# lucanest/Phyloformer

Measured on AMD Instinct MI355X. Metric: alignments/sec, 60-leaf/500-site LG+GC-like MSAs, Phyloformer forward (pf.ckpt), higher is better.
Workload: dtype f16x3-split MFMA (two fp16 limbs per operand, 3 passes), fp32 accumulate/residual

## Files before the change

### include/phyloformer_amd.h

```cpp
#ifndef PHYLOFORMER_AMD_H
#define PHYLOFORMER_AMD_H

#include <stddef.h>
#include <stdint.h>

#ifdef __cplusplus
extern "C" {
#endif

#define PF_ABI_VERSION 5

typedef enum pf_status {
    PF_OK = 0,
    PF_EINVAL = -1,
    PF_EHIP = -2,
    PF_ERCCL = -3,
    PF_ENOMEM = -4,
    PF_ESTATE = -5,
    PF_EIO = -6
} pf_status;

typedef struct pf_weights_t {
    int32_t n_blocks;
    int32_t n_heads;
// ... 73 lines not shown
int pf_bme_spr_host(const float* preds, const int32_t* start_slots, int32_t B, int32_t N, int32_t* slots, double* lengths, int32_t* steps,
                    double* tree_length, uint8_t* status);

int pf_forward_weighted(pf_handle_t* h, const uint8_t* idx, int32_t B, int32_t N, int32_t L, const float* w, float* out);
int pf_forward_weighted_device(pf_handle_t* h, const uint8_t* d_idx, int32_t B, int32_t N, int32_t L, const float* d_w,
                               float* d_out);
int pf_forward_sites_weighted(pf_handle_t* h, const uint8_t* idx, int32_t B, int32_t N, int32_t L, const int32_t* sites,
                              const float* w, int32_t S, int32_t K, float* out);
int pf_bootstrap_weighted(pf_handle_t* h, const uint8_t* idx, int32_t B, int32_t N, int32_t L, int32_t R, uint64_t seed,
                          float* out);
int pf_padded_sites(int32_t K, int32_t L);
int pf_boot_counts(int32_t L, int32_t R, uint64_t seed, int32_t r, int32_t* sites, int32_t* counts);
int pf_compress_sites(const uint8_t* idx, int32_t N, int32_t L, int32_t* first, int32_t* count);

int pf_forward_site_map(pf_handle_t* h, const uint8_t* idx, int32_t B, int32_t N, int32_t L, float* out, float* map);
int pf_forward_site_map_device(pf_handle_t* h, const uint8_t* d_idx, int32_t B, int32_t N, int32_t L, float* d_out,
                               float* d_map);
int pf_forward_site_profile(pf_handle_t* h, const uint8_t* idx, int32_t B, int32_t N, int32_t L, float* out, float* se,
                            float* profile);
int pf_site_moments_device(pf_handle_t* h, const float* d_map, int32_t B, int32_t P, int32_t L, float* d_se,
                           float* d_profile);

int pf_forward_sharded(pf_handle_t* h, const uint8_t* idx, int32_t B, int32_t N,
                       int32_t l_begin, int32_t l_end, int32_t L_total, float* out);
int pf_forward_sharded_device(pf_handle_t* h, const uint8_t* d_idx, int32_t B, int32_t N,
                              int32_t l_begin, int32_t l_end, int32_t L_total, float* d_out);

#define PF_UNIQUE_ID_BYTES 256
int pf_comm_unique_id(void* id_out);
int pf_comm_init(pf_handle_t* h, const void* unique_id, int32_t rank, int32_t world_size);
int pf_comm_destroy(pf_handle_t* h);
int pf_comm_info(char* path_out, size_t path_cap, int32_t* version);

int pf_synchronize(pf_handle_t* h);
int pf_get_stream(pf_handle_t* h, void** hip_stream_out);
int pf_device_malloc(pf_handle_t* h, size_t bytes, void** out);
int pf_device_free(pf_handle_t* h, void* p);
int pf_memcpy_h2d(pf_handle_t* h, void* dst, const void* src, size_t bytes);
int pf_memcpy_d2h(pf_handle_t* h, void* dst, const void* src, size_t bytes);

int pf_profile_reset(pf_handle_t* h);
int pf_profile_get(pf_handle_t* h, const char* kernel, int64_t* launches, double* total_ms);

int64_t pf_debug_read(pf_handle_t* h, const char* name, float* dst, int64_t cap);

int pf_device_info(pf_handle_t* h, char* name_out, size_t name_cap, int32_t* cu_count,
                   uint64_t* hbm_bytes);
int pf_device_pci(pf_handle_t* h, int32_t* domain, int32_t* bus, int32_t* device);

int pf_forward_shards_emulated(pf_handle_t* h, const uint8_t* idx, int32_t B, int32_t N, int32_t L,
                               int32_t nshards, float* out);

int pf_selftest(pf_handle_t* h, float* out);

typedef struct pf_mha_weights_t {
    int32_t n_heads;
    int32_t embed_dim;
    const float *wq, *bq, *wk, *bk, *wv, *bv, *wo, *bo;
} pf_mha_weights_t;
typedef struct pf_mha pf_mha_t;
int pf_create_bare(int device, pf_handle_t** out);
int pf_mha_create(pf_handle_t* h, const pf_mha_weights_t* w, pf_mha_t** out);
int pf_mha_destroy(pf_mha_t* m);
int pf_mha_forward(pf_mha_t* m, const float* x, int32_t B, int32_t R, int32_t C, float* y);
int pf_mha_forward_device(pf_mha_t* m, const float* d_x, int32_t B, int32_t R, int32_t C, float* d_y);

#define PF_FASTA_EBYTE (-16)
#define PF_FASTA_ERAGGED (-17)
#define PF_FASTA_ENOHEADER (-18)
#define PF_FASTA_EEMPTY (-19)
#define PF_FASTA_ECAP (-20)
#define PF_FASTA_EUTF8 (-21)
int pf_parse_fasta(const char* data, int64_t len, uint8_t* idx, int64_t idx_cap, int64_t* id_spans,
                   int32_t max_seqs, int32_t* n_out, int32_t* l_out, int64_t* detail);

int64_t pf_format_phylip(const float* preds, int32_t n, const char* const* ids, char* out, int64_t cap);
int64_t pf_format_phylip_n(const float* preds, int32_t n, const char* const* ids, const int64_t* id_lens, char* out,
                           int64_t cap);

int64_t pf_nj_newick_n(const float* preds, int32_t n, const char* const* ids, const int64_t* id_lens, int32_t clamp_negative,
                       char* out, int64_t cap);

int64_t pf_nj_format_joins_n(const int32_t* slots, const double* lengths, int32_t n, const char* const* ids, const int64_t* id_lens,
                             int32_t clamp_negative, char* out, int64_t cap);

int64_t pf_bme_newick_n(const float* preds, int32_t n, const char* const* ids, const int64_t* id_lens, int32_t clamp_negative,
                        char* out, int64_t cap);

int64_t pf_bme_spr_newick_n(const float* preds, int32_t n, const char* const* ids, const int64_t* id_lens, int32_t clamp_negative,
                            char* out, int64_t cap);

typedef struct pf_fasta_batch pf_fasta_batch_t;
int pf_fasta_batch_load(const char* const* paths, int32_t count, int32_t threads, pf_fasta_batch_t** out);
void pf_fasta_batch_free(pf_fasta_batch_t* b);
int32_t pf_fasta_batch_count(const pf_fasta_batch_t* b);
int pf_fasta_batch_infos(const pf_fasta_batch_t* b, int32_t* status, int32_t* n, int32_t* l, int64_t* detail);
int pf_fasta_batch_id(const pf_fasta_batch_t* b, int32_t file, int32_t seq, const char** id, int64_t* len);
int pf_fasta_batch_gather(const pf_fasta_batch_t* const* batches, const int32_t* file_idx, int32_t count, int32_t n,
                          int32_t l, uint8_t* dst);
int pf_phylip_write_batch(const pf_fasta_batch_t* const* batches, const int32_t* file_idx, int32_t count, int32_t n,
                          const float* preds, const char* const* out_paths, const char* const* tree_paths, int32_t threads,
                          int32_t* status);

#ifdef __cplusplus
}
#endif
// ... 2 lines not shown
```

### phyloformer_amd/csrc/pf_device.hip.h

```cpp
#pragma once
#include <hip/hip_runtime.h>
#include <stdint.h>

#include "pf_layout.h"

namespace pfk {

typedef float f32x4 __attribute__((ext_vector_type(4)));
typedef float f32x16 __attribute__((ext_vector_type(16)));
#if PF_F16
typedef _Float16 h16_t;
#define PF_MFMA(a, b, c) __builtin_amdgcn_mfma_f32_32x32x16_f16((a), (b), (c), 0, 0, 0)
#define PF_DOT2C "v_dot2c_f32_f16"
#define PF_CVT_PK "v_cvt_pk_f16_f32"
#define PF_NEG1_LO 0x0000bc00u
#define PF_NEG1_HI 0xbc000000u
#else
typedef __bf16 h16_t;
#define PF_MFMA(a, b, c) __builtin_amdgcn_mfma_f32_32x32x16_bf16((a), (b), (c), 0, 0, 0)
#define PF_DOT2C "v_dot2c_f32_bf16"
#define PF_CVT_PK "v_cvt_pk_bf16_f32"
#define PF_NEG1_LO 0x0000bf80u
#define PF_NEG1_HI 0xbf800000u
#endif
// ... 342 lines not shown
    const int k0 = (int)(((long)p * L) >> 5), k1 = (int)((((long)p + 1) * L - 1) >> 5);
    *first = (long)b * slots_aln + k0 + p;
    *count = k1 - k0 + 1;
}

template <int LO, int HI>
__device__ __forceinline__ void image_to_lds(const frag_t* src, unsigned char* smem) {
    static_assert(LO % 64 == 0 && HI % 64 == 0, "the image is copied in whole waves");
    const int wv = threadIdx.x >> 6, ln = threadIdx.x & 63;
#pragma unroll
    for (int k = 0; k < (HI - LO + MAIN_THREADS - 1) / MAIN_THREADS; ++k) {
        const int f0 = LO + k * MAIN_THREADS + wv * 64;
        if (f0 < HI) __builtin_amdgcn_global_load_lds(src + f0 + ln, smem + (size_t)f0 * 16, 16, 0, 0);
    }
}

template <int MODE, bool FLAT, bool SITEMAP = false, bool WEIGHTED = false>
__global__ void __launch_bounds__(MAIN_THREADS, MAIN_WAVES / 4) k_main(MainArgs a) {
    constexpr bool LAST = MODE == MODE_LAST || MODE == MODE_LAST_FOLD;
    constexpr bool FOLD = MODE == MODE_LAST_FOLD;
    static_assert(!SITEMAP || LAST, "the site map is the head's: last block only");
    static_assert(!WEIGHTED || (!SITEMAP && MODE != MODE_FIRST), "weighted launches: blocks' own modes, no site map");
    extern __shared__ __attribute__((aligned(16))) unsigned char smem[];
    lds_frag_t lw = (lds_frag_t)smem;
    lds_f32_t lc = (lds_f32_t)(smem + FRAG_END * 16);

    {
        const float cv = a.consts[min((int)threadIdx.x, CONST_LEN - 1)];
        if (FOLD) {
            image_to_lds<FRAG_W1, FRAG_W2>(a.wimg, smem);
            image_to_lds<FRAG_WO, FRAG_U + U_FRAGS>(a.wimg, smem);
        } else {
            image_to_lds<(MODE == MODE_FIRST) ? FRAG_WV : 0, LAST ? FRAG_WV : FRAG_END>(a.wimg, smem);
        }
        static_assert(CONST_LEN <= MAIN_THREADS, "one constant per thread");
        if (threadIdx.x < CONST_LEN) reinterpret_cast<float*>(smem + FRAG_END * 16)[threadIdx.x] = cv;
        asm volatile("s_waitcnt vmcnt(0)" ::: "memory");
    }
    __syncthreads();

    const int lane = threadIdx.x & 63;
    const int wave = __builtin_amdgcn_readfirstlane(threadIdx.x >> 6);
    const int t = lane & 31;
    const int h = lane >> 5;
    const int ntiles = (a.Lloc + 31) >> 5;
    const int ntasks = a.B * a.nt_aln;
    if (wave >= MAIN_WAVES / 2) __builtin_amdgcn_s_setprio(1);
    unsigned long long tacc[6] = {0, 0, 0, 0, 0, 0}, tprev = 0;
#define PF_TICK(k) do { if (a.prof) { const unsigned long long tn_ = __builtin_amdgcn_s_memtime(); tacc[k] += tn_ - tprev; tprev = tn_; } } while (0)
    if (a.prof) tprev = __builtin_amdgcn_s_memtime();
    lds_frag_t w1p = lw + FRAG_W1 + lane;
    lds_frag_t w2p = lw + FRAG_W2 + lane;
    lds_frag_t wop = lw + FRAG_WO + lane;
    lds_frag_t qkp = lw + FRAG_QK + h * 8 + (t & 7);
    lds_f32_t lch = lc + 4 * h;
    PF_OPAQUE(wop); PF_OPAQUE(qkp); PF_OPAQUE(lch);
    lds_frag_t wvp = wop + (FRAG_WV - FRAG_WO);
    lds_f32_t luh = (lds_f32_t)(smem + FRAG_U * 16) + 16 * h;

    {
        const int nwaves = gridDim.x * MAIN_WAVES;
#ifndef PF_RUN_MAX
#define PF_RUN_MAX 8
#endif
        const int run = max(1, min(PF_RUN_MAX, ntasks / (nwaves * 8)));
        int run0 = (blockIdx.x * MAIN_WAVES + wave) * run;
        const int task0 = run0, task1 = ntasks;
        TilePos cur = tile_pos<FLAT>(a, min(task0, ntasks - 1), ntiles);
        int frag_row = -1;
        frag_t mfr[4];
        f32x4 rqv = {0.f, 0.f, 0.f, 0.f};
        f32x4 px[8], pctx[8], pqr, pqc;
        int pri = 0, prj = 0;
        auto prefetch = [&](const TilePos& np) {
            const LanePos nl = lane_pos<FLAT>(a, np, t);
            const int ll = nl.l, pb = np.b;
            const size_t tk = nl.tok0 + nl.toff;
            if (MODE == MODE_MID0) {
                const uint8_t* ib = a.idx + (size_t)pb * a.N * a.Lloc + ll;
                const int pp = np.r0 + (nl.in_r1 ? 1 : 0);
                pri = residue(ib[(size_t)a.pair_i[pp] * a.Lloc]);
                prj = residue(ib[(size_t)a.pair_j[pp] * a.Lloc]);
            } else {
                const f32x4* xp = reinterpret_cast<const f32x4*>(a.x + tk * 64 + 4 * h);
#pragma unroll
                for (int g = 0; g < 8; ++g) px[g] = xp[2 * g];
            }
            pqr = *reinterpret_cast<const f32x4*>(a.qrow + tk * 4);
            pqc = *reinterpret_cast<const f32x4*>(a.qcol + tk * 4);
            if (MODE != MODE_FIRST) {
                int hq = h;
                asm volatile("" : "+v"(hq));
                const f32x4* cp = reinterpret_cast<const f32x4*>(a.ctx + ((size_t)pb * a.Lloc + ll) * 64 + 4 * hq);
#pragma unroll
                for (int g = 0; g < 8; ++g) pctx[g] = cp[2 * g];
            }
        };
        if (MODE != MODE_FIRST && task0 < task1) prefetch(cur);

        for (int task = task0; task < task1;) {
            const int b = cur.b;
            const int row = b * a.P + cur.r0;
            int ntask = task + 1;
            TilePos nxt = tile_next<FLAT>(a, cur);
            if (ntask == run0 + run) {
                run0 += nwaves * run;
                ntask = run0;
                if (ntask < task1) nxt = tile_pos<FLAT>(a, ntask, ntiles);
            }
            const LanePos lp = lane_pos<FLAT>(a, cur, t);
            const bool straddle = lp.wrap < 32;
            int ai = 0, aj = 0;
            if (MODE == MODE_FIRST) { const int pp = cur.r0 + (lp.in_r1 ? 1 : 0); ai = a.pair_i[pp]; aj = a.pair_j[pp]; }
            auto load_mfr = [&](int r) {
                const frag_t* mf = a.mfrag + (size_t)r * 128 + t;
#pragma unroll
                for (int q = 0; q < 4; ++q) mfr[q] = mf[q * 32];
                typedef const f32x4 __attribute__((address_space(4)))* const_f32x4_t;
                rqv = *(const_f32x4_t)(unsigned long long)(a.rq + (size_t)__builtin_amdgcn_readfirstlane(r) * 4);
                frag_row = r;
            };
            if (MODE != MODE_FIRST && row != frag_row) load_mfr(row);
            const bool valid = lp.valid;
            const int lc_ = lp.l;
            const size_t tok = lp.tok0 + lp.toff;
            float x[32];
            float zh[4] = {0.f, 0.f, 0.f, 0.f};
            float wt = 1.f;
            if (WEIGHTED && LAST) wt = a.w[(size_t)b * a.Lloc + lc_];

            if (MODE == MODE_FIRST) {
                const int ri = residue(a.idx[((size_t)b * a.N + ai) * a.Lloc + lc_]);
                const int rj = residue(a.idx[((size_t)b * a.N + aj) * a.Lloc + lc_]);
                const f32x4* ti = reinterpret_cast<const f32x4*>(a.table + ri * 64 + 4 * h);
                const f32x4* tj = reinterpret_cast<const f32x4*>(a.table + rj * 64 + 4 * h);
#pragma unroll
                for (int g = 0; g < 8; ++g) {
                    f32x4 u = ti[2 * g], w = tj[2 * g];
#pragma unroll
                    for (int i = 0; i < 4; ++i) x[4 * g + i] = u[i] + w[i];
                }
            } else {
                if (MODE == MODE_MID0) {
                    const f32x4* ti = reinterpret_cast<const f32x4*>(a.table + pri * 64 + 4 * h);
                    const f32x4* tj = reinterpret_cast<const f32x4*>(a.table + prj * 64 + 4 * h);
#pragma unroll
                    for (int g = 0; g < 8; ++g) {
                        const f32x4 u = ti[2 * g], w = tj[2 * g];
#pragma unroll
                        for (int i = 0; i < 4; ++i) x[4 * g + i] = u[i] + w[i];
                    }
                } else {
#pragma unroll
                    for (int g = 0; g < 8; ++g)
#pragma unroll
                        for (int i = 0; i < 4; ++i) x[4 * g + i] = px[g][i];
                }
                PF_TICK(0);
                if (!(a.ablate & 8)) {
                    f32x16 ya[2];
#pragma unroll
                    for (int j = 0; j < 32; ++j) ya[j >> 4][j & 15] = x[j];
                    {
                        const f32x4 qr = pqr;
                        auto mix = [&](const bool mine) {
                            float v[8];
#pragma unroll
                            for (int i = 0; i < 4; ++i) v[i] = mine ? qr[i] * rqv[i] : 0.f;
                            v[4] = v[5] = mine ? 1.f : 0.f;
                            v[6] = v[7] = 0.f;
                            frag_t qb_hi, qb_lo;
                            split8(v, qb_hi, qb_lo);
#pragma unroll
                            for (int To = 0; To < 2; ++To) mfma3(ya[To], mfr[To * 2], mfr[To * 2 + 1], qb_hi, qb_lo, To == 1);
                        };
                        mix(h == 0 && !lp.in_r1);
                        if (straddle) {
                            load_mfr(row + 1);
                            mix(h == 0 && lp.in_r1);
                        }
                    }
                    {
                        const f32x4 qc = pqc * COLAPPLY_B_SCALE;
                        float o[32];
#pragma unroll
                        for (int g = 0; g < 8; ++g) {
                            const f32x4 u = pctx[g];
#pragma unroll
                            for (int i = 0; i < 4; ++i) o[4 * g + i] = u[i] * qc[g >> 1];
                        }
#pragma unroll
                        for (int s = 0; s < 4; ++s) {
                            frag_t ob_hi, ob_lo;
                            split8(&o[8 * s], ob_hi, ob_lo);
#pragma unroll
                            for (int To = 0; To < 2; ++To) {
                                lds_frag_t f = wop + ((To * 4 + s) * 2) * 64;
                                const frag_t a_hi = f[0], a_lo = f[64];
                                mfma3(ya[To], a_hi, a_lo, ob_hi, ob_lo, To == 1);
                            }
                        }
                    }
#pragma unroll
                    for (int j = 0; j < 32; ++j) x[j] = ya[j >> 4][j & 15];
                }

                PF_TICK(1);
                if (FOLD) {
#pragma unroll
                    for (int g = 0; g < 8; ++g) {
                        const f32x4 w4 = *(lds_f32x4_t)(lch + CONST_HW + 8 * g);
#pragma unroll
                        for (int i = 0; i < 4; ++i) zh[i] = fmaf(w4[i], x[4 * g + i], zh[i]);
                    }
                }
                if (FOLD && !(a.ablate & 16)) {
                    frag_t xb_hi[4], xb_lo[4];
                    {
                        float xn[32];
                        ln_pair(x, xn);
#pragma unroll
                        for (int s = 0; s < 4; ++s) split8(&xn[8 * s], xb_hi[s], xb_lo[s]);
                    }
                    if (ntask < task1) prefetch(nxt);
                    PF_TICK(2);
#pragma unroll 1
                    for (int T = 0; T < 8; ++T) {
                        f32x16 ha;
                        lds_frag_t f1 = w1p + T * 512;
                        lds_f32_t bp = lch + CONST_B1 + 32 * T;
                        lds_f32_t up = luh + 32 * T;
                        PF_OPAQUE(f1); PF_OPAQUE(bp); PF_OPAQUE(up);
// ... 43 lines not shown
                            frag_t nh, nl;
                            if (s < 3) { nh = f1[(s + 1) * 128]; nl = f1[(s + 1) * 128 + 64]; }
                            else { nh = f2[0]; nl = f2[64]; }
                            mfma3(ha, fh, fl, xb_hi[s], xb_lo[s]);
                            fh = nh; fl = nl;
                        }
                        frag_t g_hi[2], g_lo[2];
                        gelu_split8(ha, 0, g_hi[0], g_lo[0]);
                        gelu_split8(ha, 8, g_hi[1], g_lo[1]);
#pragma unroll
                        for (int st = 0; st < 4; ++st) {
                            const int u = st >> 1, To = st & 1;
                            frag_t nh = fh, nl = fl;
                            if (st < 3) {
                                const int nu = (st + 1) >> 1, nTo = (st + 1) & 1;
                                nh = f2[(nTo * 32 + nu * 2) * 64];
                                nl = f2[(nTo * 32 + nu * 2) * 64 + 64];
                            }
                            mfma3(oa[To], fh, fl, g_hi[u], g_lo[u], To == 1);
                            fh = nh; fl = nl;
                        }
                    }
                    PF_TICK(3);
#pragma unroll
                    for (int j = 0; j < 32; ++j) x[j] = oa[j >> 4][j & 15];
                }
            }

            if (!LAST && !(a.ablate & 4)) {
                frag_t wl[8];
#pragma unroll
                for (int i = WVLO_LDS; i < 8; ++i) wl[i] = a.wv_lo[i * 64 + lane];
                if (WEIGHTED) wt = a.w[(size_t)b * a.Lloc + lc_];
                __builtin_amdgcn_sched_barrier(0);
                {
                    const size_t stok = valid ? tok : a.trash_tok + t;
                    f32x4* xo = reinterpret_cast<f32x4*>(a.x + stok * 64 + 4 * h);
#pragma unroll
                    for (int g = 0; g < 8; ++g) {
                        f32x4 u = {x[4 * g], x[4 * g + 1], x[4 * g + 2], x[4 * g + 3]};
                        xo[2 * g] = u;
                    }
                }
                if (a.ablate & 32) { cur = nxt; task = ntask; continue; }
                f32x16 va[3];
                {
                    float xn[32];
                    ln_pair(x, xn);
                    frag_t xb_hi[4], xb_lo[4];
#pragma unroll
                    for (int s = 0; s < 4; ++s) split8(&xn[8 * s], xb_hi[s], xb_lo[s]);
#pragma unroll
                    for (int s = 0; s < 4; ++s) {
                        const frag_t q_hi = qkp[(s * 2) * 16], q_lo = qkp[(s * 2 + 1) * 16];
                        if (s == 0) mfma3_zero(va[2], q_hi, q_lo, xb_hi[s], xb_lo[s]);
                        else mfma3(va[2], q_hi, q_lo, xb_hi[s], xb_lo[s]);
                    }
#pragma unroll
                    for (int s = 0; s < 4; ++s)
#pragma unroll
                        for (int T = 0; T < 2; ++T) {
                            const frag_t f_hi = wvp[(T * 4 + s) * 64];
                            const frag_t f_lo = T * 4 + s < WVLO_LDS ? wvp[(FRAG_WVLO - FRAG_WV) + (T * 4 + s) * 64] : wl[T * 4 + s];
                            if (s == 0) mfma3_zero(va[T], f_hi, f_lo, xb_hi[s], xb_lo[s], T == 1);
                            else mfma3(va[T], f_hi, f_lo, xb_hi[s], xb_lo[s], T == 1);
                        }
                }
#pragma unroll
                for (int r = 0; r < 4; ++r) va[2][r] += lc[CONST_BQK + 4 * h + r];
                float qk[4], ot[4];
#pragma unroll
                for (int i = 0; i < 4; ++i) qk[i] = elu1_fast(va[2][i]);
#pragma unroll
                for (int i = 0; i < 4; ++i) ot[i] = pair_other(qk[i], h);
                float qn[4], kn[4];
#pragma unroll
                for (int i = 0; i < 4; ++i) {
                    qn[i] = h ? ot[i] : qk[i];
                    kn[i] = h ? qk[i] : ot[i];
                }
                {
                    const size_t stok = valid ? tok : a.trash_tok + t;
                    f32x4 qs = {qn[0], qn[1], qn[2], qn[3]};
                    *reinterpret_cast<f32x4*>(a.qrow + stok * 4) = qs;
                }
                const long slot0 = (long)b * a.slots_aln + cur.kt + (FLAT ? cur.r0 : 0);
                for (int part = 0; part < (straddle ? 2 : 1); ++part) {
                    float* sp = a.spart + (size_t)(slot0 + part) * SROW;
                    const float vm = (valid && lp.in_r1 == (part == 1)) ? (WEIGHTED ? wt : 1.f) : 0.f;
                    float km[4];
#pragma unroll
                    for (int i = 0; i < 4; ++i) km[i] = kn[i] * vm;
                    {
                        float qk8[8];
#pragma unroll
                        for (int i = 0; i < 4; ++i) { qk8[i] = vm * qn[i]; qk8[4 + i] = km[i]; }
                        const float sqk = treduce8(qk8, t);
                        if (lane < 8) sp[64 + lane] = sqk;
                    }
                    {
                        float kv[32];
#pragma unroll
                        for (int j = 0; j < 32; ++j) kv[j] = km[j >> 3] * va[j >> 4][j & 15];
                        sp[kmap(t, h)] = treduce32(kv, t);
                    }
                }
            } else if (LAST) {
                float z = 0.f;
                if (FOLD) {
                    z = pair_sum((zh[0] + zh[1]) + (zh[2] + zh[3])) + lc[CONST_C0];
                } else {
#pragma unroll
                    for (int g = 0; g < 8; ++g) {
                        const f32x4 w4 = *(lds_f32x4_t)(lch + CONST_HW + 8 * g);
#pragma unroll
                        for (int i = 0; i < 4; ++i) z = fmaf(w4[i], x[4 * g + i], z);
                    }
                    z = pair_sum(z) + lc[CONST_HB];
                }
                const float spz = softplus20(z);
                const long slot0 = (long)b * a.slots_aln + cur.kt + (FLAT ? cur.r0 : 0);
                for (int part = 0; part < (straddle ? 2 : 1); ++part) {
// ... 178 lines not shown
        const float* sp = a.srow + (size_t)first * SROW;
        const int c2 = 64 + (c & 7);
        float acc = 0.f, acc2 = 0.f;
        for (int i = 0; i < nparts; i += 8) {
            const float* q0 = sp + i * SROW;
            float v[8], w8[8];
#pragma unroll
            for (int q = 0; q < 8; ++q) {
                const bool on = i + q < nparts;
                v[q] = on ? q0[q * SROW + c] : 0.f;
                w8[q] = on ? q0[q * SROW + c2] : 0.f;
            }
#pragma unroll
            for (int q = 0; q < 8; ++q) { acc += v[q]; acc2 += w8[q]; }
        }
        st[sub][c] = acc;
        if (c < 8) st[sub][64 + c] = acc2;
    }
    __syncthreads();
    if (ok) {
        const float* s = st[sub];
        const int hh = c >> 4;
        const float sk = s[68 + hh];
        ctx[sub][c] = (s[c] + bvc * sk) / sk;
        if (c < 4) {
            const float* ws = a.wst ? a.wst + (size_t)(pr / a.P) * 4 : nullptr;
            const float r = (ws ? ws[0] : a.L_total) / s[64 + c];
            rqs[sub][c] = r;
            a.rq[(size_t)pr * 4 + c] = r * (ws ? ws[2] : a.b_scale);
        }
    }
    __syncthreads();
    if (ok) {
        float* m = a.mrow ? a.mrow + (size_t)pr * MROW : nullptr;
#pragma unroll
        for (int hh = 0; hh < 4; ++hh) {
            float acc = 0.f;
#pragma unroll
            for (int d = 0; d < 16; ++d) acc = fmaf(wo[hh][d], ctx[sub][16 * hh + d], acc);
            if (m) m[hh * 64 + c] = acc * rqs[sub][hh];
            mm[sub][hh][c] = acc * (a.wst ? a.wst[(size_t)(pr / a.P) * 4 + 3] : a.a_scale);
        }
        mm[sub][4][c] = biasc;
        mm[sub][5][c] = biascol;
    }
    __syncthreads();
    if (ok) {
        const int To = c >> 5, t = c & 31;
        float v[8];
#pragma unroll
        for (int i = 0; i < 8; ++i) v[i] = (i < 6) ? mm[sub][i][32 * To + t] : 0.f;
        frag_t hi, lo;
        split8(v, hi, lo);
        frag_t* mf = a.mfrag + (size_t)pr * MFRAG_PER_PAIR + To * 64 + t;
        mf[0] = hi;
        mf[32] = lo;
    }
    }
}

__global__ void k_rowsum(const float* spart, float* srow, int npairs, int nparts_, int flat, int P, int Lloc, int slots_aln) {
    const int i = blockIdx.x * blockDim.x + threadIdx.x;
    if (i >= npairs * SROW) return;
    const int pr = i / SROW, c = i - pr * SROW;
    long first;
    int nparts;
    part_range(flat, pr, nparts_, P, Lloc, slots_aln, &first, &nparts);
    const float* sp = spart + (size_t)first * SROW + c;
    float acc = 0.f;
    for (int k = 0; k < nparts; k += 8) {
        float v[8];
#pragma unroll
        for (int q = 0; q < 8; ++q) v[q] = k + q < nparts ? sp[(size_t)(k + q) * SROW] : 0.f;
#pragma unroll
        for (int q = 0; q < 8; ++q) acc += v[q];
    }
    srow[i] = acc;
}

__global__ void k_outsum(const float* outpart, float* out, int npairs, int nparts_, float inv_L_total, int flat, int P,
                         int Lloc, int slots_aln, const float* wst) {
    const int pr = blockIdx.x * blockDim.x + threadIdx.x;
    if (pr >= npairs) return;
    long first;
    int nparts;
    part_range(flat, pr, nparts_, P, Lloc, slots_aln, &first, &nparts);
    const float* sp = outpart + first;
    float acc = 0.f;
    for (int k = 0; k < nparts; k += 8) {
        float v[8];
#pragma unroll
        for (int q = 0; q < 8; ++q) v[q] = k + q < nparts ? sp[k + q] : 0.f;
#pragma unroll
        for (int q = 0; q < 8; ++q) acc += v[q];
    }
    out[pr] = acc * (wst ? wst[(size_t)(pr / P) * 4 + 1] : inv_L_total);
}

struct ColStatsArgs {
    const float* x;
    const float* qrow;
    const float* mrow;
    float* qcol;
    float* part;
    const float* wqk;
    const float* bqk;
    const float* brow;
    int B, P, Lloc, G, nchunks;
    int sub, S, fine;
// ... 333 lines not shown
                    float v[GU][4];
#pragma unroll
                    for (int u = 0; u < GU; ++u)
#pragma unroll
                        for (int q = 0; q < 4; ++q)
                            v[u][q] = s + q < n[u] ? pg[u][(size_t)(s + q) * gs] : 0.f;
#pragma unroll
                    for (int u = 0; u < GU; ++u) t[u] = (((t[u] + v[u][0]) + v[u][1]) + v[u][2]) + v[u][3];
                }
#pragma unroll
                for (int u = 0; u < GU; ++u)
                    if (g + u < a.G) acc += t[u];
            }
        } else {
            const float* pp = a.part + ((size_t)b * a.G * a.Lloc + l) * CPART + i;
            int g = 0;
            for (; g + 4 <= a.G; g += 4) {
                const float v0 = pp[(size_t)g * gs], v1 = pp[(size_t)(g + 1) * gs], v2 = pp[(size_t)(g + 2) * gs],
                            v3 = pp[(size_t)(g + 3) * gs];
                acc = (((acc + v0) + v1) + v2) + v3;
            }
            for (; g < a.G; ++g) acc += pp[(size_t)g * gs];
        }
        zs[i] = acc;
    }
    __syncthreads();
    if (i < 256) {
        const float* z = zs + (hd >> 4) * 64 + 16 * quarter;
        float acc = 0.f;
#pragma unroll
        for (int k = 0; k < 16; ++k) acc = fmaf(w[k], z[k], acc);
        dp[quarter][hd] = acc;
    }
    __syncthreads();
    if (i < 64) {
        const int hh = hd >> 4;
        const float acc = ((dp[0][hd] + dp[1][hd]) + dp[2][hd]) + dp[3][hd];
        const float sq = zs[256 + hh], sk = zs[260 + hh];
        a.ctx[(size_t)site * 64 + hd] = (acc + a.bv[hd] * sk) / sk * (a.P / sq);
    }
}

__global__ void k_accumulate(float* dst, const float* src, size_t n) {
    const size_t i = (size_t)blockIdx.x * blockDim.x + threadIdx.x;
    if (i < n) dst[i] += src[i];
}

__global__ void k_selftest(float* out) {
    const int lane = threadIdx.x;
    out[lane] = pair_sum((float)lane);
    out[64 + lane] = pair_other((float)lane, lane >> 5);
    out[128 + lane] = row16_sum((float)lane);
    out[192 + lane] = half32_sum((float)lane);
    frag_t A1, A2, Bf;
    const int m = lane & 31, kg = lane >> 5;
#pragma unroll
    for (int i = 0; i < 8; ++i) {
        const int k = 8 * kg + i;
        A1[i] = (h16_t)(float)(m + 32 * (k % 8));
        A2[i] = (h16_t)(float)k;
        Bf[i] = (h16_t)((k == (m & 15)) ? 1.f : 0.f);
    }
    f32x16 acc1, acc2;
#pragma unroll
    for (int r = 0; r < 16; ++r) { acc1[r] = 0.f; acc2[r] = 0.f; }
    acc1 = PF_MFMA(A1, Bf, acc1);
    acc2 = PF_MFMA(A2, Bf, acc2);
#pragma unroll
    for (int r = 0; r < 16; ++r) {
        out[256 + lane * 16 + r] = acc1[r];
        out[1280 + lane * 16 + r] = acc2[r];
    }
}

#endif

}
```

### phyloformer_amd/csrc/pf_layout.h

```cpp
#pragma once

#ifndef PF_F16
#define PF_F16 1
#endif

namespace pfk {

constexpr int E = 64;
constexpr int NH = 4;
constexpr int HD = 16;
constexpr int FF = 256;
constexpr int NA = 22;
constexpr int SROW = 72;
constexpr int MROW = 4 * 64;
constexpr float LN_EPS = 1e-5f;

constexpr int FRAG_W1 = 0;
constexpr int FRAG_W2 = FRAG_W1 + 8 * 4 * 2 * 64;
constexpr int FRAG_WO = FRAG_W2 + 2 * 16 * 2 * 64;
constexpr int FRAG_WV = FRAG_WO + 2 * 4 * 2 * 64;
constexpr int FRAG_QK = FRAG_WV + 2 * 4 * 64;
#ifndef PF_WVLO_LDS
#define PF_WVLO_LDS 4
#endif
constexpr int WVLO_LDS = PF_WVLO_LDS;
constexpr int FRAG_WVLO = FRAG_QK + 4 * 2 * 16;
constexpr int FRAG_END = FRAG_WVLO + WVLO_LDS * 64;
constexpr int FRAG_U = FRAG_WV;
constexpr int U_FRAGS = FF * 4 / 16;
static_assert(FRAG_U + U_FRAGS <= FRAG_END, "the folded head fits the last block's tail");
constexpr int WVLO_FRAGS = 2 * 4 * 64;
constexpr int CONST_B1 = 0, CONST_B2 = 256, CONST_BQK = 320, CONST_HW = 328, CONST_HB = 392,
              CONST_C0 = 393, CONST_BOC = 400;
constexpr int CONST_LEN = 464;
constexpr int MAIN_LDS_BYTES = FRAG_END * 16 + CONST_LEN * 4;
constexpr int MFRAG_PER_PAIR = 2 * 2 * 32;

constexpr int MAIN_THREADS = 512;
constexpr int MAIN_WAVES = MAIN_THREADS / 64;

constexpr int PAIRTAB_ROWS = 22 * 22, PAIRTAB_W = 72;

}
```

### phyloformer_amd/csrc/pf_lib.hip

```cpp
#include <hip/hip_runtime.h>
#include <dlfcn.h>

#include <algorithm>
#include <cmath>
#include <cstdarg>
#include <cstdio>
#include <cstdlib>
#include <cstring>
#include <functional>
#include <map>
#include <mutex>
#include <string>
#include <type_traits>
#include <vector>

#include "../../include/phyloformer_amd.h"
#include "pf_device.hip.h"
#include "pf_mha.hip.h"
#include "pf_precise.hip.h"
#include "pf_generic.hip.h"
#include "pf_boot.hip.h"
#include "pf_sites.hip.h"
#include "pf_sitemap.hip.h"
#include "pf_sites_host.h"
// ... 2558 lines not shown
}

int pf_device_pci(pf_handle_t* h, int32_t* domain, int32_t* bus, int32_t* device) {
    if (!h) return PF_EINVAL;
    if (domain) *domain = h->prop.pciDomainID;
    if (bus) *bus = h->prop.pciBusID;
    if (device) *device = h->prop.pciDeviceID;
    return PF_OK;
}

int pf_forward_shards_emulated(pf_handle_t* h, const uint8_t* idx, int32_t B, int32_t N, int32_t L,
                               int32_t nshards, float* out) {
    if (!h) return PF_EINVAL;
    int rc = check_dims(h, B, N, L, L);
    if (rc) return rc;
    if (nshards < 1 || nshards > 64 || !idx || !out) return fail(h, PF_EINVAL, "bad shard count or null buffer");
    HIPCHK(h, hipSetDevice(h->device));
    if (const F64Path* f = f64_path_of(h, N, L)) return forward_shards_emulated_f64(h, *f, idx, B, N, L, nshards, out);
    if ((rc = ensure_pairs(h, N))) return rc;
    const int P = N * (N - 1) / 2;
    ShardStage stage(h);
    if ((rc = stage.upload(idx, B, N, L, nshards))) return rc;
    std::vector<ShardRun> runs;
    for (const ShardStage::Shard& s : stage.shards) {
        ShardRun r{{}, s.d_idx, nullptr, B, N, P, s.Lloc, L, tile_plan(h, P, s.Lloc), h->stream, {}};
        size_t off[WS_BUFS];
        char* ws = (char*)stage.alloc(workspace_bytes(h, B, P, r.Lloc, &r.w, off));
        r.d_out = (float*)stage.alloc((size_t)B * P * sizeof(float));
        if (!ws || !r.d_out) return fail(h, PF_ENOMEM, "shard workspace allocation failed");
        carve_workspace(ws, off, &r.w);
        runs.push_back(r);
    }
    float* total = (float*)stage.alloc((size_t)B * P * SROW * sizeof(float));
    if (!total) return fail(h, PF_ENOMEM, "shard sum buffer");
    auto reduce = [&](bool site_sums) -> int {
        const size_t count = (size_t)B * P * (site_sums ? 1 : SROW);
        for (ShardRun& r : runs)
            if (!site_sums && (rc = launch_rowsum(h, r, &r.rs))) return rc;
        hipMemsetAsync(total, 0, count * sizeof(float), h->stream);
        for (ShardRun& r : runs) {
            hipLaunchKernelGGL(k_accumulate, dim3((unsigned)((count + 255) / 256)), dim3(256), 0, h->stream,
                               total, site_sums ? r.d_out : r.w.srow, count);
            r.rs = RowStats{total, 1, 0};
        }
        return PF_OK;
    };
    rc = schedule(h, runs.data(), runs.size(), reduce);
    if (!rc && (hipMemcpyAsync(out, total, (size_t)B * P * sizeof(float), hipMemcpyDeviceToHost, h->stream) != hipSuccess ||
                hipStreamSynchronize(h->stream) != hipSuccess))
        rc = fail(h, PF_EHIP, "result copy failed");
    return rc;
}

int pf_selftest(pf_handle_t* h, float* out) {
    if (!h || !out) return PF_EINVAL;
    float* d = nullptr;
    HIPCHK(h, hipMalloc((void**)&d, 2304 * sizeof(float)));
    hipLaunchKernelGGL(k_selftest, dim3(1), dim3(64), 0, h->stream, d);
    HIPCHK(h, hipGetLastError());
    HIPCHK(h, hipMemcpyAsync(out, d, 2304 * sizeof(float), hipMemcpyDeviceToHost, h->stream));
    HIPCHK(h, hipStreamSynchronize(h->stream));
    hipFree(d);
    return PF_OK;
}

struct pf_mha {
    pf_handle* h = nullptr;
    float* wfrag = nullptr;
    float* bias = nullptr;
    char* ws = nullptr;
    size_t ws_bytes = 0;
    float* d_x = nullptr;
    float* d_y = nullptr;
    size_t d_xy_bytes = 0;
};

int pf_mha_create(pf_handle_t* h, const pf_mha_weights_t* w, pf_mha_t** out) {
    if (!h || !w || !out) return PF_EINVAL;
    if (w->n_heads != MHA_H || w->embed_dim != E)
        return fail(h, PF_EINVAL, "softmax attention kernels are specialised for embed_dim 64 / 4 heads, got %d / %d",
                    w->embed_dim, w->n_heads);
    const float* ws[4] = {w->wq, w->wk, w->wv, w->wo};
    const float* bs[4] = {w->bq, w->bk, w->bv, w->bo};
    std::vector<uint16_t> img((size_t)MHA_WTOTAL * 8);
    std::vector<float> bias(4 * E);
    for (int i = 0; i < 4; ++i) {
        if (!ws[i] || !bs[i]) return fail(h, PF_EINVAL, "pf_mha_create: NULL weight pointer");
        std::copy(bs[i], bs[i] + E, bias.begin() + i * E);
    }
    pack_frags(w->wq, E, E, E, img.data());
    pack_frags(w->wk, E, E, E, img.data() + (size_t)MHA_OFF_WK * 8);
    pack_frags(w->wv, E, E, E, img.data() + (size_t)MHA_OFF_WV * 8);
    pack_frags(w->wo, E, E, E, img.data() + (size_t)MHA_OFF_WO * 8);
    HIPCHK(h, hipSetDevice(h->device));
    pf_mha* m = new pf_mha();
    m->h = h;
    void* p = nullptr;
    if (hipMalloc(&p, img.size() * 2) != hipSuccess) { delete m; return fail(h, PF_ENOMEM, "pf_mha_create: hipMalloc failed"); }
    m->wfrag = (float*)p;
    if (hipMalloc(&p, bias.size() * 4) != hipSuccess) { hipFree(m->wfrag); delete m; return fail(h, PF_ENOMEM, "pf_mha_create: hipMalloc failed"); }
    m->bias = (float*)p;
    if (hipMemcpy(m->wfrag, img.data(), img.size() * 2, hipMemcpyHostToDevice) != hipSuccess ||
        hipMemcpy(m->bias, bias.data(), bias.size() * 4, hipMemcpyHostToDevice) != hipSuccess) {
        hipFree(m->wfrag); hipFree(m->bias); delete m;
        return fail(h, PF_EHIP, "pf_mha_create: weight upload failed");
    }
    *out = m;
    return PF_OK;
}

int pf_mha_destroy(pf_mha_t* m) {
    if (!m) return PF_OK;
    hipSetDevice(m->h->device);
    hipStreamSynchronize(m->h->stream);
    hipFree(m->wfrag); hipFree(m->bias);
    if (m->ws) hipFree(m->ws);
    if (m->d_x) hipFree(m->d_x);
// ... 82 lines not shown
```

### phyloformer_amd/engine.py

```python
from __future__ import annotations

import ctypes as C
import os
from typing import Dict, Optional, Tuple

import numpy as np

from .weights import ModelWeights

HERE = os.path.dirname(os.path.abspath(__file__))
LIB_PATH = os.path.join(HERE, "libphyloformer_amd.so")
ABI_VERSION = 5
UNIQUE_ID_BYTES = 256

PF_OK, PF_EINVAL, PF_EHIP, PF_ERCCL, PF_ENOMEM, PF_ESTATE = 0, -1, -2, -3, -4, -5


def _refuse_single_sequence(B: int, N: int):
    if N == 1 and B >= 1:
        raise RuntimeError(f"cannot reshape tensor of 0 elements into shape [{B}, -1, 0, 64] because the unspecified "
                           "dimension size -1 can be any value and is ambiguous")


class EngineError(RuntimeError):
# ... 1 lines not shown
    def __init__(self, code: int, msg: str):
        super().__init__(f"[pf status {code}] {msg}")
        self.code = code


class pf_weights_t(C.Structure):
    _fields_ = [("n_blocks", C.c_int32), ("n_heads", C.c_int32), ("embed_dim", C.c_int32),
                ("n_alphabet", C.c_int32), ("blob", C.POINTER(C.c_float)), ("blob_len", C.c_uint64)]


_H = C.c_void_p
SIGNATURES = {
    "pf_abi_version": (C.c_int, []),
    "pf_build_info": (C.c_char_p, []),
    "pf_blob_len": (C.c_uint64, [C.c_int32, C.c_int32, C.c_int32]),
    "pf_create": (C.c_int, [C.POINTER(pf_weights_t), C.c_int, C.POINTER(_H)]),
    "pf_destroy": (C.c_int, [_H]),
    "pf_last_error": (C.c_char_p, [_H]),
    "pf_set_option": (C.c_int, [_H, C.c_char_p, C.c_int64]),
    "pf_forward": (C.c_int, [_H, C.c_void_p, C.c_int32, C.c_int32, C.c_int32, C.c_void_p]),
    "pf_forward_device": (C.c_int, [_H, C.c_void_p, C.c_int32, C.c_int32, C.c_int32, C.c_void_p]),
    "pf_resample_sites_device": (C.c_int, [_H, C.c_void_p, C.c_int32, C.c_int32, C.c_int32, C.c_int32, C.c_int32,
                                           C.c_uint64, C.c_void_p]),
    "pf_bootstrap": (C.c_int, [_H, C.c_void_p, C.c_int32, C.c_int32, C.c_int32, C.c_int32, C.c_uint64, C.c_void_p]),
    "pf_window_count": (C.c_int, [C.c_int32, C.c_int32, C.c_int32]),
    "pf_window_start": (C.c_int, [C.c_int32, C.c_int32, C.c_int32, C.c_int32]),
    "pf_gather_sites_device": (C.c_int, [_H, C.c_void_p, C.c_int32, C.c_int32, C.c_int32, C.c_void_p, C.c_void_p,
                                         C.c_int32, C.c_int32, C.c_void_p]),
    "pf_forward_sites": (C.c_int, [_H, C.c_void_p, C.c_int32, C.c_int32, C.c_int32, C.c_void_p, C.c_int32, C.c_int32,
                                   C.c_void_p]),
    "pf_forward_windows": (C.c_int, [_H, C.c_void_p, C.c_int32, C.c_int32, C.c_int32, C.c_int32, C.c_int32, C.c_void_p,
                                     C.c_int32]),
    "pf_forward_sharded": (C.c_int, [_H, C.c_void_p, C.c_int32, C.c_int32, C.c_int32, C.c_int32,
                                     C.c_int32, C.c_void_p]),
    "pf_forward_sharded_device": (C.c_int, [_H, C.c_void_p, C.c_int32, C.c_int32, C.c_int32,
                                            C.c_int32, C.c_int32, C.c_void_p]),
    "pf_comm_unique_id": (C.c_int, [C.c_void_p]),
    "pf_comm_init": (C.c_int, [_H, C.c_void_p, C.c_int32, C.c_int32]),
    "pf_comm_destroy": (C.c_int, [_H]),
    "pf_comm_info": (C.c_int, [C.c_char_p, C.c_size_t, C.POINTER(C.c_int32)]),
    "pf_synchronize": (C.c_int, [_H]),
    "pf_get_stream": (C.c_int, [_H, C.POINTER(C.c_void_p)]),
    "pf_device_malloc": (C.c_int, [_H, C.c_size_t, C.POINTER(C.c_void_p)]),
    "pf_device_free": (C.c_int, [_H, C.c_void_p]),
    "pf_memcpy_h2d": (C.c_int, [_H, C.c_void_p, C.c_void_p, C.c_size_t]),
    "pf_memcpy_d2h": (C.c_int, [_H, C.c_void_p, C.c_void_p, C.c_size_t]),
    "pf_profile_reset": (C.c_int, [_H]),
    "pf_profile_get": (C.c_int, [_H, C.c_char_p, C.POINTER(C.c_int64), C.POINTER(C.c_double)]),
    "pf_debug_read": (C.c_int64, [_H, C.c_char_p, C.c_void_p, C.c_int64]),
    "pf_device_info": (C.c_int, [_H, C.c_char_p, C.c_size_t, C.POINTER(C.c_int32),
                                 C.POINTER(C.c_uint64)]),
    "pf_device_pci": (C.c_int, [_H, C.POINTER(C.c_int32), C.POINTER(C.c_int32), C.POINTER(C.c_int32)]),
    "pf_selftest": (C.c_int, [_H, C.c_void_p]),
    "pf_create_bare": (C.c_int, [C.c_int, C.POINTER(_H)]),
    "pf_mha_create": (C.c_int, [_H, C.c_void_p, C.POINTER(C.c_void_p)]),
    "pf_mha_destroy": (C.c_int, [C.c_void_p]),
    "pf_mha_forward": (C.c_int, [C.c_void_p, C.c_void_p, C.c_int32, C.c_int32, C.c_int32, C.c_void_p]),
    "pf_mha_forward_device": (C.c_int, [C.c_void_p, C.c_void_p, C.c_int32, C.c_int32, C.c_int32, C.c_void_p]),
    "pf_parse_fasta": (C.c_int, [C.c_char_p, C.c_int64, C.c_void_p, C.c_int64, C.c_void_p, C.c_int32,
                                 C.POINTER(C.c_int32), C.POINTER(C.c_int32), C.POINTER(C.c_int64)]),
    "pf_format_phylip": (C.c_int64, [C.c_void_p, C.c_int32, C.POINTER(C.c_char_p), C.c_char_p, C.c_int64]),
    "pf_format_phylip_n": (C.c_int64, [C.c_void_p, C.c_int32, C.POINTER(C.c_char_p), C.c_void_p, C.c_char_p, C.c_int64]),
    "pf_fasta_batch_load": (C.c_int, [C.POINTER(C.c_char_p), C.c_int32, C.c_int32, C.POINTER(C.c_void_p)]),
    "pf_fasta_batch_free": (None, [C.c_void_p]),
    "pf_fasta_batch_count": (C.c_int32, [C.c_void_p]),
    "pf_fasta_batch_infos": (C.c_int, [C.c_void_p, C.c_void_p, C.c_void_p, C.c_void_p, C.c_void_p]),
    "pf_fasta_batch_id": (C.c_int, [C.c_void_p, C.c_int32, C.c_int32, C.POINTER(C.c_void_p), C.POINTER(C.c_int64)]),
    "pf_fasta_batch_gather": (C.c_int, [C.c_void_p, C.c_void_p, C.c_int32, C.c_int32, C.c_int32, C.c_void_p]),
    "pf_nj_newick_n": (C.c_int64, [C.c_void_p, C.c_int32, C.POINTER(C.c_char_p), C.c_void_p, C.c_int32, C.c_char_p, C.c_int64]),
    "pf_phylip_write_batch": (C.c_int, [C.c_void_p, C.c_void_p, C.c_int32, C.c_int32, C.c_void_p,
                                        C.POINTER(C.c_char_p), C.POINTER(C.c_char_p), C.c_int32, C.c_void_p]),
    "pf_forward_shards_emulated": (C.c_int, [_H, C.c_void_p, C.c_int32, C.c_int32, C.c_int32, C.c_int32,
                                             C.c_void_p]),
    "pf_forward_site_map": (C.c_int, [_H, C.c_void_p, C.c_int32, C.c_int32, C.c_int32, C.c_void_p, C.c_void_p]),
    "pf_forward_site_map_device": (C.c_int, [_H, C.c_void_p, C.c_int32, C.c_int32, C.c_int32, C.c_void_p, C.c_void_p]),
    "pf_forward_site_profile": (C.c_int, [_H, C.c_void_p, C.c_int32, C.c_int32, C.c_int32, C.c_void_p, C.c_void_p,
                                          C.c_void_p]),
    "pf_site_moments_device": (C.c_int, [_H, C.c_void_p, C.c_int32, C.c_int32, C.c_int32, C.c_void_p, C.c_void_p]),
    "pf_gather_taxa_device": (C.c_int, [_H, C.c_void_p, C.c_int32, C.c_int32, C.c_int32, C.c_void_p, C.c_int32, C.c_int32,
                                        C.c_void_p]),
    "pf_forward_taxa": (C.c_int, [_H, C.c_void_p, C.c_int32, C.c_int32, C.c_int32, C.c_void_p, C.c_int32, C.c_int32,
                                  C.c_void_p]),
    "pf_forward_leave_one_out": (C.c_int, [_H, C.c_void_p, C.c_int32, C.c_int32, C.c_int32, C.c_void_p, C.c_void_p,
                                           C.c_void_p, C.c_void_p, C.c_void_p]),
    "pf_loo_stats_device": (C.c_int, [_H, C.c_void_p, C.c_void_p, C.c_int32, C.c_int32, C.c_void_p, C.c_void_p,
                                      C.c_void_p]),
    "pf_forward_place": (C.c_int, [_H, C.c_void_p, C.c_int32, C.c_int32, C.c_int32, C.c_int32, C.c_void_p, C.c_void_p,
                                   C.c_void_p, C.c_void_p, C.c_void_p, C.c_void_p, C.c_void_p]),
    "pf_place_stats_device": (C.c_int, [_H, C.c_void_p, C.c_void_p, C.c_void_p, C.c_int32, C.c_int32, C.c_int32,
                                        C.c_void_p, C.c_void_p, C.c_void_p, C.c_void_p]),
    "pf_forward_tiled": (C.c_int, [_H, C.c_void_p, C.c_int32, C.c_int32, C.c_int32, C.c_int32, C.c_void_p, C.c_void_p]),
    "pf_tile_combine_device": (C.c_int, [_H, C.c_void_p, C.c_int32, C.c_int32, C.c_int32, C.c_void_p, C.c_void_p]),
    "pf_tile_groups": (C.c_int, [C.c_int32, C.c_int32]),
    "pf_nj_joins": (C.c_int, [_H, C.c_void_p, C.c_int32, C.c_int32, C.c_void_p, C.c_void_p, C.c_void_p]),
    "pf_nj_joins_device": (C.c_int, [_H, C.c_void_p, C.c_int32, C.c_int32, C.c_void_p, C.c_void_p, C.c_void_p]),
    "pf_nj_format_joins_n": (C.c_int64, [C.c_void_p, C.c_void_p, C.c_int32, C.POINTER(C.c_char_p), C.c_void_p, C.c_int32,
                                         C.c_char_p, C.c_int64]),
    "pf_tile_bound": (C.c_int, [C.c_int32, C.c_int32, C.c_int32]),
    "pf_bme_nni": (C.c_int, [_H, C.c_void_p, C.c_void_p, C.c_int32, C.c_int32, C.c_void_p, C.c_void_p, C.c_void_p, C.c_void_p,
                             C.c_void_p]),
    "pf_bme_nni_device": (C.c_int, [_H, C.c_void_p, C.c_void_p, C.c_int32, C.c_int32, C.c_void_p, C.c_void_p, C.c_void_p,
                                    C.c_void_p, C.c_void_p]),
    "pf_bme_nni_host": (C.c_int, [C.c_void_p, C.c_void_p, C.c_int32, C.c_int32, C.c_void_p, C.c_void_p, C.c_void_p, C.c_void_p,
                                  C.c_void_p]),
    "pf_bme_newick_n": (C.c_int64, [C.c_void_p, C.c_int32, C.POINTER(C.c_char_p), C.c_void_p, C.c_int32, C.c_char_p, C.c_int64]),
    "pf_bme_spr": (C.c_int, [_H, C.c_void_p, C.c_void_p, C.c_int32, C.c_int32, C.c_void_p, C.c_void_p, C.c_void_p, C.c_void_p,
# ... 462 lines not shown

    def synchronize(self):
        self._check(self._lib.pf_synchronize(self._h))

    def unique_id(self) -> bytes:
        buf = C.create_string_buffer(UNIQUE_ID_BYTES)
        rc = self._lib.pf_comm_unique_id(buf)
        if rc != PF_OK:
            raise EngineError(rc, (self._lib.pf_last_error(None) or b"").decode())
        return buf.raw

    def comm_init(self, unique_id: Optional[bytes], rank: int, world: int):
        buf = C.create_string_buffer(unique_id, UNIQUE_ID_BYTES) if unique_id else None
        self._check(self._lib.pf_comm_init(self._h, buf, rank, world))
        self.rank, self.world = rank, world

    def comm_destroy(self):
        self._check(self._lib.pf_comm_destroy(self._h))
        self.rank, self.world = 0, 1

    def collective_count(self) -> int:
        return self.profile_get("collectives")[0]

    def rechecked_count(self) -> int:
        return self.profile_get("rechecked")[0]

    def comm_info(self) -> dict:
        buf = C.create_string_buffer(512)
        ver = C.c_int32()
        rc = self._lib.pf_comm_info(buf, 512, C.byref(ver))
        if rc != PF_OK:
            raise EngineError(rc, (self._lib.pf_last_error(None) or b"").decode())
        return {"library": buf.value.decode(), "version": int(ver.value)}

    def profile_reset(self):
        self._check(self._lib.pf_profile_reset(self._h))

    def profile_get(self, kernel: str) -> Tuple[int, float]:
        n = C.c_int64()
        ms = C.c_double()
        self._check(self._lib.pf_profile_get(self._h, kernel.encode(), C.byref(n), C.byref(ms)))
        return n.value, ms.value

    def debug_read(self, name: str) -> np.ndarray:
        n = self._check(self._lib.pf_debug_read(self._h, name.encode(), None, 0))
        out = np.empty(n, dtype=np.float32)
        self._check(self._lib.pf_debug_read(self._h, name.encode(), out.ctypes.data, n))
        return out

    def selftest(self) -> np.ndarray:
        out = np.empty(2304, dtype=np.float32)
        self._check(self._lib.pf_selftest(self._h, out.ctypes.data))
        return out
```

Baseline: 562.3.

## Stack hi/lo fp16 limbs along K to cut split-precision MFMA passes

Rearranges the pair-mixing fragments and QK fragments so the hi and lo limbs of the split-precision operands sit in the two K-halves of a single 32x32x16 MFMA. This replaces the three-pass mfma3 with one or two MFMAs per product. For QK, the two partial sums from the halves are added afterward. Per-pair fragment loads drop from four to two, and a selftest entry is added to check the stacked layouts. The cost is a reshuffled, more fragile fragment layout, and precision may change if any cross term is dropped.

```diff
diff --git a/include/phyloformer_amd.h b/include/phyloformer_amd.h
--- a/include/phyloformer_amd.h
+++ b/include/phyloformer_amd.h
@@ -149,6 +149,8 @@
                                int32_t nshards, float* out);
 
 int pf_selftest(pf_handle_t* h, float* out);
+#define PF_SELFTEST_STACKED_LEN 2048
+int pf_selftest_stacked(pf_handle_t* h, float* out);
 
 typedef struct pf_mha_weights_t {
     int32_t n_heads;
diff --git a/phyloformer_amd/csrc/pf_device.hip.h b/phyloformer_amd/csrc/pf_device.hip.h
--- a/phyloformer_amd/csrc/pf_device.hip.h
+++ b/phyloformer_amd/csrc/pf_device.hip.h
@@ -418,7 +418,7 @@
     lds_frag_t w1p = lw + FRAG_W1 + lane;
     lds_frag_t w2p = lw + FRAG_W2 + lane;
     lds_frag_t wop = lw + FRAG_WO + lane;
-    lds_frag_t qkp = lw + FRAG_QK + h * 8 + (t & 7);
+    lds_frag_t qkp = lw + FRAG_QK + h * 8 + (t & 7) + ((t & 8) << 1);
     lds_f32_t lch = lc + 4 * h;
     PF_OPAQUE(wop); PF_OPAQUE(qkp); PF_OPAQUE(lch);
     lds_frag_t wvp = wop + (FRAG_WV - FRAG_WO);
@@ -434,7 +434,7 @@
         const int task0 = run0, task1 = ntasks;
         TilePos cur = tile_pos<FLAT>(a, min(task0, ntasks - 1), ntiles);
         int frag_row = -1;
-        frag_t mfr[4];
+        frag_t mfr[2];
         f32x4 rqv = {0.f, 0.f, 0.f, 0.f};
         f32x4 px[8], pctx[8], pqr, pqc;
         int pri = 0, prj = 0;
@@ -479,9 +479,9 @@
             int ai = 0, aj = 0;
             if (MODE == MODE_FIRST) { const int pp = cur.r0 + (lp.in_r1 ? 1 : 0); ai = a.pair_i[pp]; aj = a.pair_j[pp]; }
             auto load_mfr = [&](int r) {
-                const frag_t* mf = a.mfrag + (size_t)r * 128 + t;
-#pragma unroll
-                for (int q = 0; q < 4; ++q) mfr[q] = mf[q * 32];
+                const frag_t* mf = a.mfrag + (size_t)r * MFRAG_PER_PAIR + 2 * t + h;
+                mfr[0] = mf[0];
+                mfr[1] = mf[64];
                 typedef const f32x4 __attribute__((address_space(4)))* const_f32x4_t;
                 rqv = *(const_f32x4_t)(unsigned long long)(a.rq + (size_t)__builtin_amdgcn_readfirstlane(r) * 4);
                 frag_row = r;
@@ -530,20 +530,23 @@
                     {
                         const f32x4 qr = pqr;
                         auto mix = [&](const bool mine) {
-                            float v[8];
+                            float v[4];
 #pragma unroll
                             for (int i = 0; i < 4; ++i) v[i] = mine ? qr[i] * rqv[i] : 0.f;
-                            v[4] = v[5] = mine ? 1.f : 0.f;
-                            v[6] = v[7] = 0.f;
-                            frag_t qb_hi, qb_lo;
-                            split8(v, qb_hi, qb_lo);
-#pragma unroll
-                            for (int To = 0; To < 2; ++To) mfma3(ya[To], mfr[To * 2], mfr[To * 2 + 1], qb_hi, qb_lo, To == 1);
+                            unsigned h01, l01, h23, l23;
+                            split_pair(v[0], v[1], h01, l01);
+                            split_pair(v[2], v[3], h23, l23);
+                            const h16x2 one2 = {(h16_t)1.f, (h16_t)1.f};
+                            const unsigned ones = mine ? __builtin_bit_cast(unsigned, one2) : 0u;
+                            const u32x4 k0 = {h01, h23, ones, ones}, k8 = {l01, l23, h01, h23};
+                            const frag_t qb = __builtin_bit_cast(frag_t, h ? k8 : k0);
+#pragma unroll
+                            for (int To = 0; To < 2; ++To) ya[To] = PF_MFMA(mfr[To], qb, ya[To]);
                         };
-                        mix(h == 0 && !lp.in_r1);
+                        mix(!lp.in_r1);
                         if (straddle) {
                             load_mfr(row + 1);
-                            mix(h == 0 && lp.in_r1);
+                            mix(lp.in_r1);
                         }
                     }
                     {
@@ -693,9 +696,10 @@
                     for (int s = 0; s < 4; ++s) split8(&xn[8 * s], xb_hi[s], xb_lo[s]);
 #pragma unroll
                     for (int s = 0; s < 4; ++s) {
-                        const frag_t q_hi = qkp[(s * 2) * 16], q_lo = qkp[(s * 2 + 1) * 16];
-                        if (s == 0) mfma3_zero(va[2], q_hi, q_lo, xb_hi[s], xb_lo[s]);
-                        else mfma3(va[2], q_hi, q_lo, xb_hi[s], xb_lo[s]);
+                        const frag_t q_st = qkp[s * 32];
+                        const f32x16 z = {0.f, 0.f, 0.f, 0.f, 0.f, 0.f, 0.f, 0.f, 0.f, 0.f, 0.f, 0.f, 0.f, 0.f, 0.f, 0.f};
+                        va[2] = PF_MFMA(q_st, xb_lo[s], s == 0 ? z : va[2]);
+                        va[2] = PF_MFMA(q_st, xb_hi[s], va[2]);
                     }
 #pragma unroll
                     for (int s = 0; s < 4; ++s)
@@ -708,7 +712,8 @@
                         }
                 }
 #pragma unroll
-                for (int r = 0; r < 4; ++r) va[2][r] += lc[CONST_BQK + 4 * h + r];
+                for (int r = 0; r < 4; ++r)
+                    va[2][r] = (va[2][r] + va[2][r + 4]) + lc[CONST_BQK + 4 * h + r];
                 float qk[4], ot[4];
 #pragma unroll
                 for (int i = 0; i < 4; ++i) qk[i] = elu1_fast(va[2][i]);
@@ -993,9 +998,11 @@
         for (int i = 0; i < 8; ++i) v[i] = (i < 6) ? mm[sub][i][32 * To + t] : 0.f;
         frag_t hi, lo;
         split8(v, hi, lo);
-        frag_t* mf = a.mfrag + (size_t)pr * MFRAG_PER_PAIR + To * 64 + t;
-        mf[0] = hi;
-        mf[32] = lo;
+        const frag_t f0 = {hi[0], hi[1], hi[2], hi[3], hi[4], hi[5], lo[4], lo[5]};
+        const frag_t f1 = {hi[0], hi[1], hi[2], hi[3], lo[0], lo[1], lo[2], lo[3]};
+        frag_t* mf = a.mfrag + (size_t)pr * MFRAG_PER_PAIR + To * 64 + 2 * t;
+        mf[0] = f0;
+        mf[1] = f1;
     }
     }
 }
@@ -1435,7 +1442,7 @@
     out[64 + lane] = pair_other((float)lane, lane >> 5);
     out[128 + lane] = row16_sum((float)lane);
     out[192 + lane] = half32_sum((float)lane);
-    frag_t A1, A2, Bf;
+    frag_t A1, A2, Bf, A3, B3, A4, B4;
     const int m = lane & 31, kg = lane >> 5;
 #pragma unroll
     for (int i = 0; i < 8; ++i) {
@@ -1443,16 +1450,24 @@
         A1[i] = (h16_t)(float)(m + 32 * (k % 8));
         A2[i] = (h16_t)(float)k;
         Bf[i] = (h16_t)((k == (m & 15)) ? 1.f : 0.f);
-    }
-    f32x16 acc1, acc2;
-#pragma unroll
-    for (int r = 0; r < 16; ++r) { acc1[r] = 0.f; acc2[r] = 0.f; }
+        A3[i] = (h16_t)(float)(m < 8 ? m + 1 : m < 16 ? 57 + m : 0);
+        B3[i] = (h16_t)((k == 0) ? 1.f : 0.f);
+        A4[i] = (h16_t)(float)(k + 1 + 16 * (m & 3));
+        B4[i] = (h16_t)((i == (m & 7)) ? (kg ? 64.f : 1.f) : 0.f);
+    }
+    f32x16 acc1, acc2, acc3, acc4;
+#pragma unroll
+    for (int r = 0; r < 16; ++r) { acc1[r] = 0.f; acc2[r] = 0.f; acc3[r] = 0.f; acc4[r] = 0.f; }
     acc1 = PF_MFMA(A1, Bf, acc1);
     acc2 = PF_MFMA(A2, Bf, acc2);
+    acc3 = PF_MFMA(A3, B3, acc3);
+    acc4 = PF_MFMA(A4, B4, acc4);
 #pragma unroll
     for (int r = 0; r < 16; ++r) {
         out[256 + lane * 16 + r] = acc1[r];
         out[1280 + lane * 16 + r] = acc2[r];
+        out[2304 + lane * 16 + r] = acc3[r];
+        out[3328 + lane * 16 + r] = acc4[r];
     }
 }
 
diff --git a/phyloformer_amd/csrc/pf_layout.h b/phyloformer_amd/csrc/pf_layout.h
--- a/phyloformer_amd/csrc/pf_layout.h
+++ b/phyloformer_amd/csrc/pf_layout.h
@@ -34,7 +34,7 @@
               CONST_C0 = 393, CONST_BOC = 400;
 constexpr int CONST_LEN = 464;
 constexpr int MAIN_LDS_BYTES = FRAG_END * 16 + CONST_LEN * 4;
-constexpr int MFRAG_PER_PAIR = 2 * 2 * 32;
+constexpr int MFRAG_PER_PAIR = 2 * 32 * 2;
 
 constexpr int MAIN_THREADS = 512;
 constexpr int MAIN_WAVES = MAIN_THREADS / 64;
diff --git a/phyloformer_amd/csrc/pf_lib.hip b/phyloformer_amd/csrc/pf_lib.hip
--- a/phyloformer_amd/csrc/pf_lib.hip
+++ b/phyloformer_amd/csrc/pf_lib.hip
@@ -2634,17 +2634,20 @@
     return rc;
 }
 
-int pf_selftest(pf_handle_t* h, float* out) {
+static int selftest_range(pf_handle_t* h, float* out, int first, int count) {
     if (!h || !out) return PF_EINVAL;
+    constexpr int total = 2304 + PF_SELFTEST_STACKED_LEN;
     float* d = nullptr;
-    HIPCHK(h, hipMalloc((void**)&d, 2304 * sizeof(float)));
+    HIPCHK(h, hipMalloc((void**)&d, total * sizeof(float)));
     hipLaunchKernelGGL(k_selftest, dim3(1), dim3(64), 0, h->stream, d);
     HIPCHK(h, hipGetLastError());
-    HIPCHK(h, hipMemcpyAsync(out, d, 2304 * sizeof(float), hipMemcpyDeviceToHost, h->stream));
+    HIPCHK(h, hipMemcpyAsync(out, d + first, (size_t)count * sizeof(float), hipMemcpyDeviceToHost, h->stream));
     HIPCHK(h, hipStreamSynchronize(h->stream));
     hipFree(d);
     return PF_OK;
 }
+int pf_selftest(pf_handle_t* h, float* out) { return selftest_range(h, out, 0, 2304); }
+int pf_selftest_stacked(pf_handle_t* h, float* out) { return selftest_range(h, out, 2304, PF_SELFTEST_STACKED_LEN); }
 
 struct pf_mha {
     pf_handle* h = nullptr;
diff --git a/phyloformer_amd/engine.py b/phyloformer_amd/engine.py
--- a/phyloformer_amd/engine.py
+++ b/phyloformer_amd/engine.py
@@ -77,6 +77,7 @@
                                  C.POINTER(C.c_uint64)]),
     "pf_device_pci": (C.c_int, [_H, C.POINTER(C.c_int32), C.POINTER(C.c_int32), C.POINTER(C.c_int32)]),
     "pf_selftest": (C.c_int, [_H, C.c_void_p]),
+    "pf_selftest_stacked": (C.c_int, [_H, C.c_void_p]),
     "pf_create_bare": (C.c_int, [C.c_int, C.POINTER(_H)]),
     "pf_mha_create": (C.c_int, [_H, C.c_void_p, C.POINTER(C.c_void_p)]),
     "pf_mha_destroy": (C.c_int, [C.c_void_p]),
@@ -645,3 +646,8 @@
         out = np.empty(2304, dtype=np.float32)
         self._check(self._lib.pf_selftest(self._h, out.ctypes.data))
         return out
+
+    def selftest_stacked(self) -> np.ndarray:
+        out = np.empty(2048, dtype=np.float32)
+        self._check(self._lib.pf_selftest_stacked(self._h, out.ctypes.data))
+        return out
```

Result: no change. 567.7 (median of 6 runs) (+1.0%).
